# ufal/neuralmonkey

Hardware: AMD Instinct MI355X
Metric: target tokens/sec/node (train), 512-hid GRU+attn (higher is better)
Workload: dtype f32; 1 GPU; translation.ini-shape: biGRU-512 enc + Bahdanau attn + GRU-512 dec, B=128/GPU, src_len=tgt_len=50, V=32000, weights N(0,0.05)/orthogonal (BASELINE.md 3), CrossEntropyTrainer(l2=1e-8, clip_norm=1.0) + Adam(1e-4), one optimizer step per step, 8 distinct HBM-resident batches in rotation; global_batch=128, seq_len=50, parallelism=dp1

## Files before the change

neuralmonkey_amd/csrc/nm_gemm.hip:

```cpp
#include <atomic>

#include "nm_common.h"

#include <stdlib.h>

typedef float f32x16 __attribute__((ext_vector_type(16)));

bool nm_medium_gemm(hipStream_t st, int transB, long M, long N, long K, const float* A, long lda, const float* B,
                    long ldb, float* C, long ldc, const float* bias, int act, int accumulate);

struct GemmArgs {
    const float* A;
    const float* B;
    float* C;
    const float* bias;
    int M, N, K;
    long lda, ldb, ldc;
    long sA, sB, sC;
    int act;
    int accumulate;
    float* ws;
    int splitk;
    int swizzle;
    float* stats;
    int store_c;
    int prio;
    const float* const* ptrs;
    int chain_k;
};

__device__ __forceinline__ float apply_act(float x, int act) {
    if (act == 1) return nm_tanh(x);
    if (act == 2) return fmaxf(x, 0.0f);
    return x;
}

__device__ __forceinline__ void store_tile32(const GemmArgs& g, float* __restrict__ C,
                                             const f32x16& acc, int m0, int n0, int lane) {
    const int col = n0 + (lane & 31);
    if (col >= g.N) return;
    const float bv = g.bias ? g.bias[col] : 0.0f;
#pragma unroll
    for (int r = 0; r < 16; ++r) {
        const int row = m0 + (r & 3) + 8 * (r >> 2) + 4 * (lane >> 5);
        if (row < g.M) {
            float* p = C + (long)row * g.ldc + col;
            float v = acc[r] + bv;
            if (g.accumulate) v += *p;
            *p = apply_act(v, g.act);
        }
    }
}

template <int WM, int WN, int TM, int TN, bool TA, bool TB, bool VEC, int BK, bool STATS = false, int PF = 1,
          int NCH = 1, bool CHAIN = false>
__global__ __launch_bounds__(WM * WN * 64) void gemm_tiled(GemmArgs g, int tiles_m) {
    static_assert(!CHAIN || (TA && !TB && VEC && !STATS), "chained K: the weight-gradient form only");
    constexpr int NT = WM * WN * 64;
    constexpr int BM = WM * 32 * TM, BN = WN * 32 * TN;
    constexpr int LA = BM * BK / 4 / NT, LB = BN * BK / 4 / NT, KQ = BK / 4;
    static_assert(LA >= 1 && LB >= 1 && LA * NT * 4 == BM * BK && LB * NT * 4 == BN * BK, "tile / thread mismatch");
    constexpr int LDAS = BM + 4, LDBS = BN + 4;
    constexpr int A_FLOATS = 2 * BK * LDAS, B_FLOATS = 2 * BK * LDBS;
    constexpr int ST_ROWS = BM > 256 ? 128 : BM / 2;
    constexpr int ST_FLOATS = STATS ? ST_ROWS * (BN + 1) + 3 * NT : 0;
    constexpr int SM_FLOATS = A_FLOATS + B_FLOATS > ST_FLOATS ? A_FLOATS + B_FLOATS : ST_FLOATS;
    static_assert((A_FLOATS * 4) % 16 == 0, "B tile must stay 16-byte aligned");
    __shared__ __attribute__((aligned(16))) float smem[SM_FLOATS];
    float (*As)[BK][LDAS] = reinterpret_cast<float (*)[BK][LDAS]>(smem);
    float (*Bs)[BK][LDBS] = reinterpret_cast<float (*)[BK][LDBS]>(smem + A_FLOATS);

    const int tid = threadIdx.x, lane = tid & 63, wave = tid >> 6;
    int bm, bn;
    {
        const int npid = (int)gridDim.x;
        int pid = (int)blockIdx.x;
        if (g.swizzle) {
            const int per = npid / 8, rem = npid % 8, x = pid % 8, i = pid / 8;
            pid = x * per + (x < rem ? x : rem) + i;
            constexpr int GROUP_M = 8;
            const int tiles_n = npid / tiles_m;
            const int width = GROUP_M * tiles_n;
            const int group = pid / width, first = group * GROUP_M;
            const int gsz = (tiles_m - first) < GROUP_M ? (tiles_m - first) : GROUP_M;
            bm = first + (pid % width) % gsz;
            bn = (pid % width) / gsz;
        } else {
            bm = pid % tiles_m;
            bn = pid / tiles_m;
        }
    }
    const int m0 = bm * BM, n0 = bn * BN;
    const float* __restrict__ A = (g.ptrs && !CHAIN) ? g.ptrs[3 * blockIdx.z] : g.A + (long)blockIdx.z * g.sA;
    const float* __restrict__ B = (g.ptrs && !CHAIN) ? g.ptrs[3 * blockIdx.z + 1] : g.B + (long)blockIdx.z * g.sB;
    float* __restrict__ C = (g.ptrs && !CHAIN) ? const_cast<float*>(g.ptrs[3 * blockIdx.z + 2]) : g.C + (long)blockIdx.z * g.sC;

    float4 ra0[LA], rb0[LB], ra1[PF == 2 ? LA : 1], rb1[PF == 2 ? LB : 1];

    auto load_a = [&](int k0, float4* ra) {
#pragma unroll
        for (int it = 0; it < LA; ++it) {
            const int idx = tid + it * NT;
            int m, k;
            if (TA) { k = idx / (BM / 4); m = (idx % (BM / 4)) * 4; }
            else    { m = idx / KQ;       k = (idx % KQ) * 4; }
            const int gm = m0 + m, gk = k0 + k;
            float4 v = make_float4(0.f, 0.f, 0.f, 0.f);
            if (TA) {
                const float* p = A + (long)gk * g.lda + gm;
                if constexpr (CHAIN) {
                    const int mem = k0 / g.chain_k;
                    p = g.ptrs[3 * mem] + (long)(gk - mem * g.chain_k) * g.lda + gm;
                }
                if (gk < g.K) {
                    if (VEC) { if (gm < g.M) v = *reinterpret_cast<const float4*>(p); }
                    else {
                        if (gm + 0 < g.M) v.x = p[0];
                        if (gm + 1 < g.M) v.y = p[1];
                        if (gm + 2 < g.M) v.z = p[2];
                        if (gm + 3 < g.M) v.w = p[3];
                    }
                }
            } else {
                const float* p = A + (long)gm * g.lda + gk;
                if (gm < g.M) {
                    if (VEC) { if (gk < g.K) v = *reinterpret_cast<const float4*>(p); }
                    else {
                        if (gk + 0 < g.K) v.x = p[0];
                        if (gk + 1 < g.K) v.y = p[1];
                        if (gk + 2 < g.K) v.z = p[2];
                        if (gk + 3 < g.K) v.w = p[3];
                    }
                }
            }
            ra[it] = v;
        }
    };
    auto load_b = [&](int k0, float4* rb) {
#pragma unroll
        for (int it = 0; it < LB; ++it) {
            const int idx = tid + it * NT;
            int n, k;
            if (!TB) { k = idx / (BN / 4); n = (idx % (BN / 4)) * 4; }
            else     { n = idx / KQ;       k = (idx % KQ) * 4; }
            const int gn = n0 + n, gk = k0 + k;
            float4 v = make_float4(0.f, 0.f, 0.f, 0.f);
            if (!TB) {
                const float* p = B + (long)gk * g.ldb + gn;
                if constexpr (CHAIN) {
                    const int mem = k0 / g.chain_k;
                    p = g.ptrs[3 * mem + 1] + (long)(gk - mem * g.chain_k) * g.ldb + gn;
                }
                if (gk < g.K) {
                    if (VEC) { if (gn < g.N) v = *reinterpret_cast<const float4*>(p); }
                    else {
                        if (gn + 0 < g.N) v.x = p[0];
                        if (gn + 1 < g.N) v.y = p[1];
                        if (gn + 2 < g.N) v.z = p[2];
                        if (gn + 3 < g.N) v.w = p[3];
                    }
                }
            } else {
                const float* p = B + (long)gn * g.ldb + gk;
                if (gn < g.N) {
                    if (VEC) { if (gk < g.K) v = *reinterpret_cast<const float4*>(p); }
                    else {
                        if (gk + 0 < g.K) v.x = p[0];
                        if (gk + 1 < g.K) v.y = p[1];
                        if (gk + 2 < g.K) v.z = p[2];
                        if (gk + 3 < g.K) v.w = p[3];
                    }
                }
            }
            rb[it] = v;
// ... 154 lines not shown
        float* psum = pmax + 2 * NT;
        bool okj[TN];
#pragma unroll
        for (int j = 0; j < TN; ++j) {
            const int col = n0 + wn + j * 32 + (lane & 31);
            okj[j] = col < g.N;
            const float bv = (okj[j] && g.bias) ? g.bias[col] : 0.0f;
#pragma unroll
            for (int i = 0; i < TM; ++i)
#pragma unroll
                for (int r = 0; r < 16; ++r) acc[i][j][r] += bv;
        }
        const int tiles_n = (int)gridDim.x / tiles_m;
        const int rr = tid % HR, q = tid / HR;
        for (int h = 0; h < NP; ++h) {
            __syncthreads();
#pragma unroll
            for (int i = 0; i < TM; ++i) {
                const int rbase = wm + i * 32 - h * HR;
                if (rbase >= 0 && rbase < HR) {
#pragma unroll
                    for (int j = 0; j < TN; ++j)
#pragma unroll
                        for (int r = 0; r < 16; ++r)
                            T[(rbase + (r & 3) + 8 * (r >> 2) + 4 * (lane >> 5)) * TS + wn + j * 32 + (lane & 31)] =
                                okj[j] ? acc[i][j][r] : -INFINITY;
                }
            }
            __syncthreads();
            const float* trow = T + rr * TS + q * CW;
            float best = -INFINITY;
            int bi = 0x7fffffff;
#pragma unroll
            for (int c = 0; c < CW; ++c) {
                const float v = trow[c];
                if (v > best) { best = v; bi = n0 + q * CW + c; }
            }
            pmax[q * HR + rr] = best;
            parg[q * HR + rr] = bi;
            __syncthreads();
            float m = pmax[rr];
#pragma unroll
            for (int w = 1; w < TPR; ++w) m = fmaxf(m, pmax[w * HR + rr]);
            float sum = 0.0f;
#pragma unroll
            for (int c = 0; c < CW; ++c) sum += expf(trow[c] - m);
            psum[q * HR + rr] = sum;
            __syncthreads();
            const int row = m0 + h * HR + tid;
            if (tid < HR && row < g.M) {
                float tot = psum[tid];
                int a = parg[tid];
#pragma unroll
                for (int w = 1; w < TPR; ++w) {
                    tot += psum[w * HR + tid];
                }
                float bm = pmax[tid];
#pragma unroll
                for (int w = 1; w < TPR; ++w)
                    if (pmax[w * HR + tid] > bm) { bm = pmax[w * HR + tid]; a = parg[w * HR + tid]; }
                float4 rec;
                rec.x = bm; rec.y = tot; rec.z = __int_as_float(a); rec.w = 0.0f;
                *reinterpret_cast<float4*>(g.stats + ((long)row * tiles_n + bn) * 4) = rec;
            }
        }
        if (!g.store_c) return;
        GemmArgs gs = g;
        gs.bias = nullptr;
#pragma unroll
        for (int i = 0; i < TM; ++i)
#pragma unroll
            for (int j = 0; j < TN; ++j)
                store_tile32(gs, C, acc[i][j], m0 + wm + i * 32, n0 + wn + j * 32, lane);
        return;
    }
    if (!g.store_c) return;
#pragma unroll
    for (int i = 0; i < TM; ++i)
#pragma unroll
        for (int j = 0; j < TN; ++j)
            store_tile32(g, C, acc[i][j], m0 + wm + i * 32, n0 + wn + j * 32, lane);
}

__global__ void splitk_reduce(GemmArgs g) {
    const long idx = (long)blockIdx.x * blockDim.x + threadIdx.x;
    const long total = (long)g.M * g.N;
    if (idx >= total) return;
    const int row = (int)(idx / g.N), col = (int)(idx - (long)row * g.N);
    float s = 0.0f;
    for (int k = 0; k < g.splitk; ++k) s += g.ws[(long)k * total + idx];
    float* p = g.C + (long)row * g.ldc + col;
    float v = s + (g.bias ? g.bias[col] : 0.0f);
    if (g.accumulate) v += *p;
    *p = apply_act(v, g.act);
}

#include "nm_gru.h"

__device__ __forceinline__ void gru_epilogue(const GruEpi& e, int d, int row, int col, float s) {
    const int H = e.H;
    const long ro = (long)d * e.R + row;
    int pos, ppos;
    const bool live = gru_epi_pos(e, row, d, e.t, pos, ppos);
    if (e.mode == 1) {
        float gate = 0.0f;
        if (live) gate = nm_sigmoid(e.xp[d * e.x_dir + (long)row * e.x_row + (long)pos * e.x_time + col] + s);
        e.ru[ro * 2 * H + col] = gate;
        if (col < H) e.rh[ro * H + col] = live ? gate * e.h_in[ro * H + col] : 0.0f;
    } else if (e.mode == 2) {
        const float hp = e.h_in[ro * H + col];
        if (!live) {
            if (e.h_out != e.h_in) e.h_out[ro * H + col] = hp;
            if (e.c_save) e.c_save[ro * H + col] = 0.0f;
            return;
        }
        const float c = nm_tanh(e.xp[d * e.x_dir + (long)row * e.x_row + (long)pos * e.x_time + 2 * H + col] + s);
        const float u = e.ru[ro * 2 * H + H + col];
        const float hn = u * hp + (1.0f - u) * c;
        e.h_out[ro * H + col] = hn;
        if (e.c_save) e.c_save[ro * H + col] = c;
        if (e.out) e.out[d * e.o_dir + (long)row * e.o_row + (long)pos * e.o_time + col] = hn;
    } else if (e.mode == 3) {
        if (!live) { e.dgpre[ro * 2 * H + col] = 0.0f; return; }
        const float rr = e.ru[ro * 2 * H + col];
        const float hp = gru_epi_hprev(e, ro, d, row, e.t, ppos, col);
        const float drp = s * hp * rr * (1.0f - rr);
        e.dh[ro * H + col] += s * rr;
        e.dgpre[ro * 2 * H + col] = drp;
        e.dxp[d * e.dx_dir + (long)row * e.dx_row + (long)pos * e.dx_time + col] = drp;
    } else {
        if (!live) {
            e.dh[ro * H + col] = s;
            e.dcpre[ro * H + col] = 0.0f;
            e.dgpre[ro * 2 * H + H + col] = 0.0f;
            return;
        }
        float dhv = s;
        if (e.dout) dhv += e.dout[d * e.do_dir + (long)row * e.do_row + (long)pos * e.do_time + col];
        const float u = e.ru[ro * 2 * H + H + col];
        const float c = e.c[ro * H + col];
        const float hp = gru_epi_hprev(e, ro, d, row, e.t, ppos, col);
        const float dcp = dhv * (1.0f - u) * (1.0f - c * c);
        const float dup = dhv * (hp - c) * u * (1.0f - u);
        e.dh[ro * H + col] = dhv * u;
        e.dcpre[ro * H + col] = dcp;
        e.dgpre[ro * 2 * H + H + col] = dup;
        float* dx = e.dxp + d * e.dx_dir + (long)row * e.dx_row + (long)pos * e.dx_time;
        dx[H + col] = dup;
        dx[2 * H + col] = dcp;
    }
}

struct GruPre {
    float a, b, c, d;
    int pos, ppos;
    bool live;
};

__device__ __forceinline__ GruPre gru_epi_load(const GruEpi& e, int d, int row, int col, const float* __restrict__ C,
                                               long ldc, bool accumulate) {
    GruPre q;
    q.a = q.b = q.c = q.d = 0.0f;
    const int H = e.H;
    const long ro = (long)d * e.R + row;
    q.live = gru_epi_pos(e, row, d, e.t, q.pos, q.ppos);
    if (e.mode == 1) {
// ... 483 lines not shown
    if (pad > 0) {
        const unsigned ok_bit = 1u << (nm_cur()->device & 15), bad_bit = ok_bit << 16;
        unsigned seen = devs.load(std::memory_order_relaxed);
        if (!(seen & (ok_bit | bad_bit))) {
            const bool ok = hipFuncSetAttribute((const void*)kern, hipFuncAttributeMaxDynamicSharedMemorySize,
                                                NM_GEMM_BG_MAX_PAD) == hipSuccess;
            if (!ok) (void)hipGetLastError();
            seen = devs.fetch_or(ok ? ok_bit : bad_bit, std::memory_order_relaxed) | (ok ? ok_bit : bad_bit);
        }
        if ((seen & bad_bit) && pad > 30 * 1024) pad = 30 * 1024;
    }
    hipLaunchKernelGGL(kern, grid, block, (size_t)pad, st, args...);
}

static inline int bg_lds_target() {
    const int cap = nm_cur()->sw.gemm_bg_wgs;
    return (cap >= 1 && cap <= 3) ? 160 * 1024 / (cap + 1) + 512 : 0;
}

static void launch_skinny(const GemmArgs& g_in, int batch, bool tb, const GruEpi& epi, hipStream_t st) {
    GemmArgs g = g_in;
    const bool background = nm_cur()->sw.background != 0;
    g.prio = background ? 0 : nm_cur()->sw.step_prio;
    const int want = background ? bg_lds_target() : 0;
    const int K = g.K;
    const bool no16 = nm_cur()->sw.gemm_no16;
    if (!no16 && K >= 256 && (long)nm_cdiv(g.M, 32) * nm_cdiv(g.N, 32) * batch < 256) {
        const int tiles_m = nm_cdiv(g.M, 16), tiles_n = nm_cdiv(g.N, 16);
        dim3 grid(tiles_m * tiles_n, 1, (unsigned)batch);
        static const bool wide = !(getenv("NM_SKINNY16_WIDE") && atoi(getenv("NM_SKINNY16_WIDE")) == 0);
        const long ntiles = (long)tiles_m * tiles_n * batch;
        const int ks = (K >= 512 && !(wide && ntiles > 512)) ? 16 : 8;
        static DevMask devs16[4];
#define NM_GS16(KS_, I_)                                                                                               \
    do {                                                                                                               \
        const int pad = bg_pad(want, KS_ * 1024);                                                                      \
        if (tb) launch_padded(gemm_skinny16<KS_, true>, devs16[I_], pad, grid, dim3(KS_ * 64), st, g, tiles_m, epi);   \
        else launch_padded(gemm_skinny16<KS_, false>, devs16[I_ + 1], pad, grid, dim3(KS_ * 64), st, g, tiles_m, epi); \
    } while (0)
        if (ks == 16) NM_GS16(16, 0);
        else NM_GS16(8, 2);
#undef NM_GS16
        return;
    }
    const int tiles_m = nm_cdiv(g.M, 32), tiles_n = nm_cdiv(g.N, 32);
    dim3 grid(tiles_m * tiles_n, 1, (unsigned)batch);
    const int ks = (K >= 512) ? 16 : (K >= 256 ? 8 : (K >= 128 ? 4 : 1));
    static DevMask devs32[8];
#define NM_GS(KS_, I_)                                                                                               \
    do {                                                                                                             \
        const int pad = bg_pad(want, KS_ * 4096);                                                                    \
        if (tb) launch_padded(gemm_skinny<KS_, true>, devs32[I_], pad, grid, dim3(KS_ * 64), st, g, tiles_m, epi);   \
        else launch_padded(gemm_skinny<KS_, false>, devs32[I_ + 1], pad, grid, dim3(KS_ * 64), st, g, tiles_m, epi); \
    } while (0)
    if (ks == 16) NM_GS(16, 0);
    else if (ks == 8) NM_GS(8, 2);
    else if (ks == 4) NM_GS(4, 4);
    else NM_GS(1, 6);
#undef NM_GS
}

template <int WM, int WN, int TM, int TN, int BK, int PF = 1, int NCH = 1>
static void launch_tiled(const GemmArgs& g, int batch, bool ta, bool tb, bool vec, hipStream_t st, int pad_lds = 0) {
    const int tiles_m = nm_cdiv(g.M, WM * 32 * TM), tiles_n = nm_cdiv(g.N, WN * 32 * TN);
    dim3 grid(tiles_m * tiles_n, g.splitk, batch), block(WM * WN * 64);
    static DevMask attr_devs[8];
#define NM_GT(TA_, TB_, V_)                                                                              \
    launch_padded(gemm_tiled<WM, WN, TM, TN, TA_, TB_, V_, BK, false, PF, NCH>,                         \
                  attr_devs[(TA_ ? 4 : 0) + (TB_ ? 2 : 0) + (V_ ? 1 : 0)], pad_lds, grid, block, st, g, tiles_m)
    if (vec) {
        if (!ta && !tb) NM_GT(false, false, true);
        else if (!ta && tb) NM_GT(false, true, true);
        else if (ta && !tb) NM_GT(true, false, true);
        else NM_GT(true, true, true);
    } else {
        if (!ta && !tb) NM_GT(false, false, false);
        else if (!ta && tb) NM_GT(false, true, false);
        else if (ta && !tb) NM_GT(true, false, false);
        else NM_GT(true, true, false);
    }
#undef NM_GT
}

extern "C" int nm_gemm_f32(void* stream, int transA, int transB, int64_t M, int64_t N, int64_t K,
                           const float* A, int64_t lda, const float* B, int64_t ldb, float* C,
                           int64_t ldc, const float* bias, int act, int accumulate, int64_t batch,
                           int64_t strideA, int64_t strideB, int64_t strideC, int algo,
                           void* workspace, int64_t workspace_bytes) {
    NM_REQUIRE(A && B && C, "nm_gemm_f32: null operand");
    NM_REQUIRE(M >= 0 && N >= 0 && K >= 0 && batch >= 1, "nm_gemm_f32: bad shape %ld %ld %ld x%ld",
               (long)M, (long)N, (long)K, (long)batch);
    NM_REQUIRE(act >= 0 && act <= 2, "nm_gemm_f32: bad act %d", act);
    NM_REQUIRE(M < (1 << 30) && N < (1 << 30) && K < (1 << 30), "nm_gemm_f32: dim too large");
    if (M == 0 || N == 0) return NM_OK;
    NM_REQUIRE(K > 0, "nm_gemm_f32: K == 0");
    GemmArgs g{A, B, C, bias, (int)M, (int)N, (int)K, (long)lda, (long)ldb, (long)ldc,
               (long)strideA, (long)strideB, (long)strideC, act, accumulate, nullptr, 1, 0, nullptr, 1};
    const NmSwitches& sw = nm_cur()->sw;
    const int swz_env = sw.gemm_swz;
    g.swizzle = swz_env;
    const bool nostore = sw.gemm_nostore;
    if (nostore) g.store_c = 0;
    hipStream_t st = nm_stream(stream);
    const bool ta = transA != 0, tb = transB != 0;
    if (algo == 0 && !sw.background && !ta && batch == 1 && !nostore &&
        nm_medium_gemm(st, transB, M, N, K, A, lda, B, ldb, C, ldc, bias, act, accumulate)) {
        NM_LAUNCH_CHECK("nm_gemm_f32 (medium)");
    }

    const bool a_vec = nm_aligned16(A) && lda % 4 == 0 && strideA % 4 == 0 && ((ta ? M : K) % 4 == 0);
    const bool b_vec = nm_aligned16(B) && ldb % 4 == 0 && strideB % 4 == 0 && ((tb ? K : N) % 4 == 0);
    const bool vec = a_vec && b_vec;

    int bg_lds = 0;
    if (algo == 4 || (algo == 0 && sw.background)) {
        algo = 0;
        bg_lds = bg_lds_target();
    }
    bool skinny_ok = !ta && a_vec && K % 8 == 0 && (!tb || b_vec);
    int pick = algo;
    if (pick == 0) {
        const long blocks128 = (long)nm_cdiv(M, 128) * nm_cdiv(N, 128) * batch;
        if (skinny_ok && M <= 256 && (long)N * K <= (4L << 20)) pick = 3;
        else if (blocks128 >= 512) pick = 1;
        else pick = 2;
    }
    if (pick == 3) {
        NM_REQUIRE(skinny_ok, "nm_gemm_f32: skinny path needs transA=0, aligned A, K%%8==0");
        launch_skinny(g, (int)batch, tb, GruEpi{}, st);
    } else {
        if (workspace && batch == 1 && K >= 1024) {
            const bool big = (algo == 1) || (algo == 0 && M >= 128 && N >= 128);
            const int tile = big ? 128 : 64;
            const long tiles = (long)nm_cdiv(M, tile) * nm_cdiv(N, tile);
            const int sk_env = sw.gemm_sk;
            const long nkt = (K + 15) / 16;
            const double kt_us = big ? 0.95 : 0.30;
            long best_sk = 1;
            double best = 1e30;
            for (long sk = 1; sk <= 16; ++sk) {
                if (sk > 1 && (K / sk < 128 || sk * M * N * (long)sizeof(float) > workspace_bytes)) break;
                const long blocks = tiles * sk;
                const long rounds = (blocks + 255) / 256;
                const double per_cu = (double)blocks / 256.0;
                const double thin = per_cu <= 1.0 ? 1.35 : (per_cu <= 2.0 ? 1.15 : 1.0);
                double cost = (double)rounds * (double)((nkt + sk - 1) / sk) * kt_us * thin;
                if (sk > 1) cost += (double)(sk + 1) * M * N * 4.0 / 3.0e6 + 3.0;
                if (cost < best) { best = cost; best_sk = sk; }
            }
            if (sk_env > 0 && sk_env <= 16 && K / sk_env >= 128 &&
                (long)sk_env * M * N * (long)sizeof(float) <= workspace_bytes) best_sk = sk_env;
            if (best_sk >= 2) {
                g.splitk = (int)best_sk;
                g.ws = reinterpret_cast<float*>(workspace);
                if (algo == 0) pick = big ? 1 : 2;
            }
        }
        const int cfg_env = sw.gemm_cfg;
        if (pick == 1) {
            if (bg_lds > 0 && sw.gemm_bg_cfg == 2) launch_tiled<4, 2, 2, 2, 16>(g, (int)batch, ta, tb, vec, st, bg_pad(bg_lds, 50176));
            else if (cfg_env == 1) launch_tiled<4, 2, 1, 2, 16>(g, (int)batch, ta, tb, vec, st, bg_pad(bg_lds, 33792));
            else if (cfg_env == 3) launch_tiled<4, 4, 1, 1, 32>(g, (int)batch, ta, tb, vec, st);
            else if (cfg_env == 4) launch_tiled<4, 2, 1, 2, 32>(g, (int)batch, ta, tb, vec, st);
            else if (cfg_env == 5) launch_tiled<2, 4, 2, 1, 16>(g, (int)batch, ta, tb, vec, st);
            else if (cfg_env == 2) launch_tiled<4, 2, 2, 2, 16>(g, (int)batch, ta, tb, vec, st);
            else if (cfg_env == 6) launch_tiled<4, 2, 1, 2, 16, 2>(g, (int)batch, ta, tb, vec, st);
            else if (cfg_env == 7) launch_tiled<4, 2, 2, 2, 16, 2>(g, (int)batch, ta, tb, vec, st);
            else if (cfg_env == 8) launch_tiled<2, 2, 2, 2, 16, 2>(g, (int)batch, ta, tb, vec, st);
            else if (cfg_env == 9) launch_tiled<4, 2, 1, 2, 32, 2>(g, (int)batch, ta, tb, vec, st);
            else launch_tiled<2, 2, 2, 2, 16>(g, (int)batch, ta, tb, vec, st);
        } else if (sw.gemm_cfg64 == 1 && bg_lds == 0 && g.splitk == 1) {
            launch_tiled<2, 1, 2, 2, 16>(g, (int)batch, ta, tb, vec, st);
        } else if (sw.gemm_cfg64 == 2 && bg_lds == 0 && g.splitk == 1) {
            launch_tiled<1, 2, 2, 2, 16>(g, (int)batch, ta, tb, vec, st);
        } else if (sw.gemm_cfg64 == 3 && bg_lds == 0 && g.splitk == 1) {
            launch_tiled<2, 2, 2, 2, 16>(g, (int)batch, ta, tb, vec, st);
        } else if (sw.gemm_chains == 4) {
            launch_tiled<2, 2, 1, 1, 16, 1, 4>(g, (int)batch, ta, tb, vec, st);
        } else if (sw.gemm_chains == 2) {
            launch_tiled<2, 2, 1, 1, 16, 1, 2>(g, (int)batch, ta, tb, vec, st);
        } else {
            launch_tiled<2, 2, 1, 1, 16>(g, (int)batch, ta, tb, vec, st, bg_pad(bg_lds, 17408));
        }
        if (g.splitk > 1) {
            const long total = (long)M * N;
            hipLaunchKernelGGL(splitk_reduce, dim3(nm_cdiv(total, 256)), dim3(256), 0, st, g);
        }
    }
    NM_LAUNCH_CHECK("nm_gemm_f32");
}

extern "C" int nm_gemm_f32_group(void* stream, int transA, int transB, int64_t M, int64_t N, int64_t K,
                                 const void* pointer_table, int64_t lda, int64_t ldb, int64_t ldc, int accumulate,
                                 int64_t count) {
    NM_REQUIRE(pointer_table && count >= 1 && count < 65536, "nm_gemm_f32_group: null table / bad count %ld", (long)count);
    NM_REQUIRE(M > 0 && N > 0 && K > 0 && M < (1 << 30) && N < (1 << 30) && K < (1 << 30),
               "nm_gemm_f32_group: bad shape %ld %ld %ld", (long)M, (long)N, (long)K);
    const bool ta = transA != 0, tb = transB != 0;
    NM_REQUIRE(lda % 4 == 0 && ldb % 4 == 0 && ldc % 4 == 0 && (ta ? M : K) % 4 == 0 && (tb ? K : N) % 4 == 0,
               "nm_gemm_f32_group: leading dimensions and contiguous extents must be multiples of 4 (the operands "
               "themselves 16-byte aligned)");
    GemmArgs g{nullptr, nullptr, nullptr, nullptr, (int)M, (int)N, (int)K, (long)lda, (long)ldb, (long)ldc,
               0, 0, 0, 0, accumulate, nullptr, 1, 0, nullptr, 1};
    g.swizzle = nm_cur()->sw.gemm_swz;
    g.ptrs = reinterpret_cast<const float* const*>(pointer_table);
    hipStream_t st = nm_stream(stream);
    const long blocks128 = (long)nm_cdiv(M, 128) * nm_cdiv(N, 128) * count;
    if (blocks128 >= 192) launch_tiled<4, 2, 1, 2, 16>(g, (int)count, ta, tb, true, st);
    else launch_tiled<2, 2, 1, 1, 16>(g, (int)count, ta, tb, true, st);
    NM_LAUNCH_CHECK("nm_gemm_f32_group");
}

extern "C" int nm_gemm_f32_chain(void* stream, int64_t M, int64_t N, int64_t rows, int64_t count,
                                 const void* pointer_table, int64_t lda, int64_t ldb, float* C, int64_t ldc,
                                 int accumulate, void* workspace, int64_t workspace_bytes) {
    NM_REQUIRE(pointer_table && C && count >= 1 && count < 65536, "nm_gemm_f32_chain: null pointer / bad count %ld", (long)count);
    NM_REQUIRE(M > 0 && N > 0 && rows > 0 && rows % 16 == 0 && rows * count < (1 << 30) && M < (1 << 30) && N < (1 << 30),
               "nm_gemm_f32_chain: bad shape M=%ld N=%ld rows=%ld (a multiple of 16) x %ld", (long)M, (long)N, (long)rows,
               (long)count);
    NM_REQUIRE(lda % 4 == 0 && ldb % 4 == 0 && M % 4 == 0 && N % 4 == 0,
               "nm_gemm_f32_chain: leading dimensions and M, N must be multiples of 4 (the operands 16-byte aligned)");
    const long K = rows * count;
    GemmArgs g{nullptr, nullptr, C, nullptr, (int)M, (int)N, (int)K, (long)lda, (long)ldb, (long)ldc,
               0, 0, 0, 0, accumulate, nullptr, 1, 0, nullptr, 1};
    g.swizzle = nm_cur()->sw.gemm_swz;
    g.ptrs = reinterpret_cast<const float* const*>(pointer_table);
    g.chain_k = (int)rows;
    const bool big = M >= 128 && N >= 128;
    const int tile = big ? 128 : 64;
    const long tiles = (long)nm_cdiv(M, tile) * nm_cdiv(N, tile);
    if (workspace && K >= 1024) {
        const long nkt = (K + 15) / 16;
        const double kt_us = big ? 0.95 : 0.30;
        long best_sk = 1;
        double best = 1e30;
        for (long sk = 1; sk <= 16; ++sk) {
            if (sk > 1 && (K / sk < 128 || sk * M * N * (long)sizeof(float) > workspace_bytes)) break;
            const long blocks = tiles * sk;
            const long rounds = (blocks + 255) / 256;
            const double per_cu = (double)blocks / 256.0;
            const double thin = per_cu <= 1.0 ? 1.35 : (per_cu <= 2.0 ? 1.15 : 1.0);
            double cost = (double)rounds * (double)((nkt + sk - 1) / sk) * kt_us * thin;
            if (sk > 1) cost += (double)(sk + 1) * M * N * 4.0 / 3.0e6 + 3.0;
            if (cost < best) { best = cost; best_sk = sk; }
// ... 103 lines not shown
```

neuralmonkey_amd/csrc/nm_host.hip:

```cpp
#include "nm_common.h"
#include "../../include/nmhip.h"

#include <mutex>
#include <stdlib.h>

#define NM_CTX_MAGIC 0x4e4d4358u

static int env_int(const char* name, int dflt) {
    const char* e = getenv(name);
    return e ? atoi(e) : dflt;
}

static void switches_from_env(NmSwitches* sw) {
    sw->attn_maxrows = env_int("NM_ATTN_MAXROWS", 12);
    if (sw->attn_maxrows < 1 || sw->attn_maxrows > 16) sw->attn_maxrows = 12;
    sw->attn_nomerge = getenv("NM_ATTN_NOMERGE") != nullptr;
    sw->attn_nofast = getenv("NM_ATTN_NOFAST") != nullptr;
    sw->attn_whole = getenv("NM_ATTN_WHOLE") ? (env_int("NM_ATTN_WHOLE", 0) != 0 ? 1 : 0) : -1;
    sw->aeb_wide_off = getenv("NM_AEB_WIDE") && env_int("NM_AEB_WIDE", 1) == 0;
    sw->gemm_no16 = getenv("NM_GEMM_NO16") != nullptr;
    sw->gemm_swz = env_int("NM_GEMM_SWZ", 1);
    sw->gemm_nostore = getenv("NM_GEMM_NOSTORE") != nullptr;
    sw->gemm_sk = env_int("NM_GEMM_SK", 0);
    sw->gemm_cfg = env_int("NM_GEMM_CFG", 1);
    sw->gemm_chains = env_int("NM_GEMM_CHAINS", 1);
    sw->gemm_cfg64 = env_int("NM_GEMM_CFG64", 0);
    sw->gemm_bg_wgs = env_int("NM_GEMM_BG_WGS", 1);
    sw->gemm_bg_cfg = env_int("NM_GEMM_BG_CFG", 1);
    sw->background = 0;
    sw->step_prio = env_int("NM_STEP_PRIO", 1);
    sw->stats_cfg = env_int("NM_STATS_CFG", 3);
    sw->stats_ablate = getenv("NM_STATS_ABLATE") != nullptr;
    sw->beam_ns = env_int("NM_BEAM_NS", 0);
    sw->sdp_mfma = !(getenv("NM_SDP_MFMA") && env_int("NM_SDP_MFMA", 1) == 0);
    sw->medium_m = env_int("NM_STEP_MEDIUM", 1);
    sw->sdp_decode = !(getenv("NM_SDP_DECODE") && env_int("NM_SDP_DECODE", 1) == 0);
}

static NmCtx* ctx_new(int device) {
    NmCtx* c = new NmCtx();
    c->magic = NM_CTX_MAGIC;
    c->device = device;
    switches_from_env(&c->sw);
    c->prof_on = false;
    c->prof_used = 0;
    return c;
}

static thread_local NmCtx* t_bound = nullptr;
static NmCtx* g_default = nullptr;
static std::once_flag g_default_once;

NmCtx* nm_cur() {
    if (t_bound) return t_bound;
    std::call_once(g_default_once, [] {
        int dev = 0;
        if (hipGetDevice(&dev) != hipSuccess) dev = 0;
        g_default = ctx_new(dev);
    });
    return g_default;
}

std::pair<hipEvent_t, hipEvent_t>* nm_prof_next_pair(NmCtx* c) {
    if (c->prof_used == c->prof_pool.size()) {
        hipEvent_t a, b;
        if (hipEventCreate(&a) != hipSuccess || hipEventCreate(&b) != hipSuccess) return nullptr;
        c->prof_pool.emplace_back(a, b);
    }
    return &c->prof_pool[c->prof_used++];
}

static NmCtx* ctx_of(void* handle) {
    if (!handle) return nm_cur();
    NmCtx* c = static_cast<NmCtx*>(handle);
    return c->magic == NM_CTX_MAGIC ? c : nullptr;
}

extern "C" int nm_create(int device, void** out_ctx) {
    NM_REQUIRE(out_ctx, "nm_create: null output pointer");
    if (device < 0) {
        int dev = 0;
        if (hipGetDevice(&dev) != hipSuccess) dev = 0;
        device = dev;
    }
    *out_ctx = ctx_new(device);
    return NM_OK;
}

extern "C" int nm_destroy(void* ctx) {
    NM_REQUIRE(ctx, "nm_destroy: null context");
    NmCtx* c = static_cast<NmCtx*>(ctx);
    NM_REQUIRE(c->magic == NM_CTX_MAGIC, "nm_destroy: not a context (or destroyed twice)");
    NM_REQUIRE(c != g_default, "nm_destroy: the default context belongs to the library");
    if (t_bound == c) t_bound = nullptr;
    for (auto& pr : c->prof_pool) {
        (void)hipEventDestroy(pr.first);
        (void)hipEventDestroy(pr.second);
    }
    c->magic = 0;
    delete c;
    return NM_OK;
}

extern "C" int nm_ctx_bind(void* ctx) {
    if (!ctx) {
        t_bound = nullptr;
        return NM_OK;
// ... 103 lines not shown
```

Baseline: 603,800 tokens/s.

## Add three-stage LDS ring GEMM kernel and make it the default config

Adds a new 128x128 GEMM kernel, 512 threads, BK=16, that keeps a three-stage shared-memory ring. Global loads for a future tile, LDS stores for the next tile and MFMA on the current tile are interleaved with a single barrier per stage, and fragment reads are double-buffered and ordered with sched_group_barrier hints. The default NM_GEMM_CFG moves to 10, so the ring kernel replaces the previous 4x2x1x2 tiled kernel on the pick-1 path, including background launches. It also factors out the block-to-tile swizzle into a shared helper and adds algo==5 as a way to force the old loop. The aim is to hide memory latency better than the previous double-buffered loop, at the cost of more LDS per block and a waves-per-EU occupancy target that may limit registers.

```diff
diff --git a/neuralmonkey_amd/csrc/nm_gemm.hip b/neuralmonkey_amd/csrc/nm_gemm.hip
--- a/neuralmonkey_amd/csrc/nm_gemm.hip
+++ b/neuralmonkey_amd/csrc/nm_gemm.hip
@@ -52,6 +52,25 @@
     }
 }
 
+__device__ __forceinline__ void tile_of_block(const GemmArgs& g, int tiles_m, int& bm, int& bn) {
+    const int npid = (int)gridDim.x;
+    int pid = (int)blockIdx.x;
+    if (g.swizzle) {
+        const int per = npid / 8, rem = npid % 8, x = pid % 8, i = pid / 8;
+        pid = x * per + (x < rem ? x : rem) + i;
+        constexpr int GROUP_M = 8;
+        const int tiles_n = npid / tiles_m;
+        const int width = GROUP_M * tiles_n;
+        const int group = pid / width, first = group * GROUP_M;
+        const int gsz = (tiles_m - first) < GROUP_M ? (tiles_m - first) : GROUP_M;
+        bm = first + (pid % width) % gsz;
+        bn = (pid % width) / gsz;
+    } else {
+        bm = pid % tiles_m;
+        bn = pid / tiles_m;
+    }
+}
+
 template <int WM, int WN, int TM, int TN, bool TA, bool TB, bool VEC, int BK, bool STATS = false, int PF = 1,
           int NCH = 1, bool CHAIN = false>
 __global__ __launch_bounds__(WM * WN * 64) void gemm_tiled(GemmArgs g, int tiles_m) {
@@ -72,24 +91,7 @@
 
     const int tid = threadIdx.x, lane = tid & 63, wave = tid >> 6;
     int bm, bn;
-    {
-        const int npid = (int)gridDim.x;
-        int pid = (int)blockIdx.x;
-        if (g.swizzle) {
-            const int per = npid / 8, rem = npid % 8, x = pid % 8, i = pid / 8;
-            pid = x * per + (x < rem ? x : rem) + i;
-            constexpr int GROUP_M = 8;
-            const int tiles_n = npid / tiles_m;
-            const int width = GROUP_M * tiles_n;
-            const int group = pid / width, first = group * GROUP_M;
-            const int gsz = (tiles_m - first) < GROUP_M ? (tiles_m - first) : GROUP_M;
-            bm = first + (pid % width) % gsz;
-            bn = (pid % width) / gsz;
-        } else {
-            bm = pid % tiles_m;
-            bn = pid / tiles_m;
-        }
-    }
+    tile_of_block(g, tiles_m, bm, bn);
     const int m0 = bm * BM, n0 = bn * BN;
     const float* __restrict__ A = (g.ptrs && !CHAIN) ? g.ptrs[3 * blockIdx.z] : g.A + (long)blockIdx.z * g.sA;
     const float* __restrict__ B = (g.ptrs && !CHAIN) ? g.ptrs[3 * blockIdx.z + 1] : g.B + (long)blockIdx.z * g.sB;
@@ -410,6 +412,144 @@
             store_tile32(g, C, acc[i][j], m0 + wm + i * 32, n0 + wn + j * 32, lane);
 }
 
+template <bool VEC>
+__device__ __forceinline__ float4 ring_load4(const float* __restrict__ p, bool line_ok, int c, int c_end) {
+    float4 v = make_float4(0.f, 0.f, 0.f, 0.f);
+    if (line_ok) {
+        if (VEC) { if (c < c_end) v = *reinterpret_cast<const float4*>(p); }
+        else {
+            if (c + 0 < c_end) v.x = p[0];
+            if (c + 1 < c_end) v.y = p[1];
+            if (c + 2 < c_end) v.z = p[2];
+            if (c + 3 < c_end) v.w = p[3];
+        }
+    }
+    return v;
+}
+
+static constexpr int NM_RING_LDS_BYTES = 3 * 2 * 16 * (128 + 4) * 4;
+static constexpr bool NM_RING_BACKGROUND = true;
+
+template <bool TA, bool TB, bool VEC>
+__global__ __launch_bounds__(512) __attribute__((amdgpu_waves_per_eu(6))) void gemm_ring(GemmArgs g, int tiles_m) {
+    constexpr int BM = 128, BN = 128, BK = 16, KQ = BK / 4, TN = 2, NS = 3;
+    constexpr int LDS_ROW = BM + 4;
+    constexpr int STAGE = 2 * BK * LDS_ROW;
+    static_assert(NS * STAGE * 4 == NM_RING_LDS_BYTES && (BK * LDS_ROW * 4) % 16 == 0, "ring layout");
+    __shared__ __attribute__((aligned(16))) float smem[NS * STAGE];
+
+    const int tid = threadIdx.x, lane = tid & 63, wave = tid >> 6;
+    int bm, bn;
+    tile_of_block(g, tiles_m, bm, bn);
+    const int m0 = bm * BM, n0 = bn * BN;
+    const float* __restrict__ A = g.A + (long)blockIdx.z * g.sA;
+    const float* __restrict__ B = g.B + (long)blockIdx.z * g.sB;
+    float* __restrict__ C = g.C + (long)blockIdx.z * g.sC;
+
+    const int nkt_all = (g.K + BK - 1) / BK;
+    const int per_slice = (nkt_all + g.splitk - 1) / g.splitk;
+    const int kt0 = blockIdx.y * per_slice;
+    const int n = min(nkt_all, kt0 + per_slice) - kt0;
+
+    const int ka = TA ? tid / (BM / 4) : (tid % KQ) * 4, ma = TA ? (tid % (BM / 4)) * 4 : tid / KQ;
+    const int kb = !TB ? tid / (BN / 4) : (tid % KQ) * 4, nb = !TB ? (tid % (BN / 4)) * 4 : tid / KQ;
+    const int gma = m0 + ma, gnb = n0 + nb;
+    int gka = kt0 * BK + ka, gkb = kt0 * BK + kb;
+    const float* pa = TA ? A + (long)gka * g.lda + gma : A + (long)gma * g.lda + gka;
+    const float* pb = !TB ? B + (long)gkb * g.ldb + gnb : B + (long)gnb * g.ldb + gkb;
+    const long step_a = TA ? BK * g.lda : BK, step_b = !TB ? BK * g.ldb : BK;
+    const int sa = ka * LDS_ROW + ma, sb = BK * LDS_ROW + kb * LDS_ROW + nb;
+
+    auto load_tile = [&](float4& ra, float4& rb) {
+        ra = TA ? ring_load4<VEC>(pa, gka < g.K, gma, g.M) : ring_load4<VEC>(pa, gma < g.M, gka, g.K);
+        rb = !TB ? ring_load4<VEC>(pb, gkb < g.K, gnb, g.N) : ring_load4<VEC>(pb, gnb < g.N, gkb, g.K);
+        pa += step_a; pb += step_b;
+        gka += BK; gkb += BK;
+    };
+    auto store_stage = [&](int s, const float4& ra, const float4& rb) {
+        float* S = smem + s * STAGE;
+        if (TA) *reinterpret_cast<float4*>(S + sa) = ra;
+        else {
+            S[sa + 0 * LDS_ROW] = ra.x;
+            S[sa + 1 * LDS_ROW] = ra.y;
+            S[sa + 2 * LDS_ROW] = ra.z;
+            S[sa + 3 * LDS_ROW] = ra.w;
+        }
+        if (!TB) *reinterpret_cast<float4*>(S + sb) = rb;
+        else {
+            S[sb + 0 * LDS_ROW] = rb.x;
+            S[sb + 1 * LDS_ROW] = rb.y;
+            S[sb + 2 * LDS_ROW] = rb.z;
+            S[sb + 3 * LDS_ROW] = rb.w;
+        }
+    };
+
+    f32x16 acc[TN];
+#pragma unroll
+    for (int j = 0; j < TN; ++j)
+#pragma unroll
+        for (int r = 0; r < 16; ++r) acc[j][r] = 0.0f;
+
+    const int wm = (wave / 2) * 32, wn = (wave % 2) * 32 * TN;
+    const int fa = (lane >> 5) * LDS_ROW + wm + (lane & 31), fb = BK * LDS_ROW + (lane >> 5) * LDS_ROW + wn + (lane & 31);
+    float a[2], b[2][TN];
+    auto read_frag = [&](int s, int kk, int p) {
+        const float* S = smem + s * STAGE + kk * LDS_ROW;
+        a[p] = S[fa];
+#pragma unroll
+        for (int j = 0; j < TN; ++j) b[p][j] = S[fb + j * 32];
+    };
+    auto mma_tile = [&](int cur, int nxt) {
+#pragma unroll
+        for (int kk = 0; kk < BK; kk += 2) {
+            const int p = (kk >> 1) & 1;
+            if (kk + 2 < BK) read_frag(cur, kk + 2, p ^ 1);
+            else read_frag(nxt, 0, p ^ 1);
+#pragma unroll
+            for (int j = 0; j < TN; ++j) acc[j] = __builtin_amdgcn_mfma_f32_32x32x2f32(a[p], b[p][j], acc[j], 0, 0, 0);
+            __builtin_amdgcn_sched_group_barrier(0x100, 1 + TN, 0);
+            __builtin_amdgcn_sched_group_barrier(0x008, TN, 0);
+        }
+    };
+
+    if (n > 0) {
+        float4 ra, rb;
+        {
+            float4 ra1, rb1;
+            load_tile(ra, rb);
+            if (n > 1) load_tile(ra1, rb1);
+            store_stage(0, ra, rb);
+            if (n > 2) load_tile(ra, rb);
+            if (n > 1) store_stage(1, ra1, rb1);
+        }
+        __syncthreads();
+        read_frag(0, 0, 0);
+        int t = 0;
+        while (t < n) {
+#pragma unroll
+            for (int s = 0; s < NS; ++s) {
+                if (t + 2 < n) store_stage((s + 2) % NS, ra, rb);
+                if (t + 3 < n) load_tile(ra, rb);
+                mma_tile(s, (s + 1) % NS);
+                __syncthreads();
+                if (++t >= n) break;
+            }
+        }
+    }
+
+    if (g.splitk > 1) {
+        GemmArgs gs = g;
+        gs.ldc = g.N; gs.bias = nullptr; gs.act = 0; gs.accumulate = 0;
+        float* slab = g.ws + (long)blockIdx.y * g.M * g.N;
+#pragma unroll
+        for (int j = 0; j < TN; ++j) store_tile32(gs, slab, acc[j], m0 + wm, n0 + wn + j * 32, lane);
+        return;
+    }
+    if (!g.store_c) return;
+#pragma unroll
+    for (int j = 0; j < TN; ++j) store_tile32(g, C, acc[j], m0 + wm, n0 + wn + j * 32, lane);
+}
+
 __global__ void splitk_reduce(GemmArgs g) {
     const long idx = (long)blockIdx.x * blockDim.x + threadIdx.x;
     const long total = (long)g.M * g.N;
@@ -1059,6 +1199,27 @@
 #undef NM_GT
 }
 
+static void launch_ring(const GemmArgs& g, int batch, bool ta, bool tb, bool vec, hipStream_t st, int pad_lds = 0) {
+    const int tiles_m = nm_cdiv(g.M, 128), tiles_n = nm_cdiv(g.N, 128);
+    dim3 grid(tiles_m * tiles_n, g.splitk, batch), block(512);
+    static DevMask attr_devs[8];
+#define NM_GR(TA_, TB_, V_)                                                                              \
+    launch_padded(gemm_ring<TA_, TB_, V_>, attr_devs[(TA_ ? 4 : 0) + (TB_ ? 2 : 0) + (V_ ? 1 : 0)], pad_lds, grid, \
+                  block, st, g, tiles_m)
+    if (vec) {
+        if (!ta && !tb) NM_GR(false, false, true);
+        else if (!ta && tb) NM_GR(false, true, true);
+        else if (ta && !tb) NM_GR(true, false, true);
+        else NM_GR(true, true, true);
+    } else {
+        if (!ta && !tb) NM_GR(false, false, false);
+        else if (!ta && tb) NM_GR(false, true, false);
+        else if (ta && !tb) NM_GR(true, false, false);
+        else NM_GR(true, true, false);
+    }
+#undef NM_GR
+}
+
 extern "C" int nm_gemm_f32(void* stream, int transA, int transB, int64_t M, int64_t N, int64_t K,
                            const float* A, int64_t lda, const float* B, int64_t ldb, float* C,
                            int64_t ldc, const float* bias, int act, int accumulate, int64_t batch,
@@ -1089,6 +1250,8 @@
     const bool b_vec = nm_aligned16(B) && ldb % 4 == 0 && strideB % 4 == 0 && ((tb ? K : N) % 4 == 0);
     const bool vec = a_vec && b_vec;
 
+    const bool old_loop = algo == 5;
+    if (old_loop) algo = 1;
     int bg_lds = 0;
     if (algo == 4 || (algo == 0 && sw.background)) {
         algo = 0;
@@ -1136,7 +1299,9 @@
         const int cfg_env = sw.gemm_cfg;
         if (pick == 1) {
             if (bg_lds > 0 && sw.gemm_bg_cfg == 2) launch_tiled<4, 2, 2, 2, 16>(g, (int)batch, ta, tb, vec, st, bg_pad(bg_lds, 50176));
-            else if (cfg_env == 1) launch_tiled<4, 2, 1, 2, 16>(g, (int)batch, ta, tb, vec, st, bg_pad(bg_lds, 33792));
+            else if (cfg_env == 10 && !old_loop && (bg_lds == 0 || NM_RING_BACKGROUND))
+                launch_ring(g, (int)batch, ta, tb, vec, st, bg_pad(bg_lds, NM_RING_LDS_BYTES));
+            else if (cfg_env == 1 || cfg_env == 10 || old_loop) launch_tiled<4, 2, 1, 2, 16>(g, (int)batch, ta, tb, vec, st, bg_pad(bg_lds, 33792));
             else if (cfg_env == 3) launch_tiled<4, 4, 1, 1, 32>(g, (int)batch, ta, tb, vec, st);
             else if (cfg_env == 4) launch_tiled<4, 2, 1, 2, 32>(g, (int)batch, ta, tb, vec, st);
             else if (cfg_env == 5) launch_tiled<2, 4, 2, 1, 16>(g, (int)batch, ta, tb, vec, st);
diff --git a/neuralmonkey_amd/csrc/nm_host.hip b/neuralmonkey_amd/csrc/nm_host.hip
--- a/neuralmonkey_amd/csrc/nm_host.hip
+++ b/neuralmonkey_amd/csrc/nm_host.hip
@@ -22,7 +22,7 @@
     sw->gemm_swz = env_int("NM_GEMM_SWZ", 1);
     sw->gemm_nostore = getenv("NM_GEMM_NOSTORE") != nullptr;
     sw->gemm_sk = env_int("NM_GEMM_SK", 0);
-    sw->gemm_cfg = env_int("NM_GEMM_CFG", 1);
+    sw->gemm_cfg = env_int("NM_GEMM_CFG", 10);
     sw->gemm_chains = env_int("NM_GEMM_CHAINS", 1);
     sw->gemm_cfg64 = env_int("NM_GEMM_CFG64", 0);
     sw->gemm_bg_wgs = env_int("NM_GEMM_BG_WGS", 1);
```

Result: faster. 621,200 tokens/s (median of 6 runs) (+2.9%).
